# fboehm/DBSLMM

Hardware: AMD Instinct MI355X
Metric: SNPs solved/sec (whole node) + max-|Δβ| vs CPU ref, 1M SNP × 10k indiv (higher is better)
Workload: dtype f64

## Files before the change

dbslmm_amd/_lib.py:

```python
from __future__ import annotations

import ctypes as C
import os

HERE = os.path.dirname(os.path.abspath(__file__))
LIB_PATH = os.path.join(HERE, "libdbslmm_hip.so")

EXPORTS = (
    "dbslmm_abi_version", "dbslmm_ctx_create", "dbslmm_ctx_destroy", "dbslmm_last_error",
    "dbslmm_est", "dbslmm_plan_create", "dbslmm_plan_run", "dbslmm_plan_sync",
    "dbslmm_plan_download", "dbslmm_plan_set_sigma", "dbslmm_plan_destroy", "dbslmm_plan_run_multi",
    "dbslmm_plan_enable_timing", "dbslmm_plan_kernel_ms", "dbslmm_plan_workload",
    "dbslmm_bed_maf", "dbslmm_read_snp_std", "dbslmm_valid_blocks", "dbslmm_plan_variance",
    "dbslmm_ctx_create_multi", "dbslmm_ctx_num_devices", "dbslmm_plan_shard_info",
    "dbslmm_ctx_cache_bed", "dbslmm_ctx_cache_bed_fd", "dbslmm_plan_block_matrix",
    "dbslmm_shard_plan", "dbslmm_plan_create_units", "dbslmm_shard_plan_problem",
    "dbslmm_plan_block_iters", "dbslmm_bed_row_stats", "dbslmm_out_ranges", "dbslmm_plan_score",
    "dbslmm_ld_r2", "dbslmm_clump", "dbslmm_ld_scores", "dbslmm_ldsc_fit",
)

ABI_VERSION = 21
K_UNPACK, K_GRAM, K_CHOL_LARGE, K_CHOL_SMALL, K_CHOL_TILED, K_TRSV, K_PCG, K_PCG_BLOCK = 0, 1, 2, 3, 4, 5, 6, 7
KERNEL_NAMES = ("dbslmm_unpack_stats", "dbslmm_gram", "dbslmm_chol_large", "dbslmm_chol_small",
                "dbslmm_tchol", "dbslmm_trsv", "dbslmm_pcg", "dbslmm_pcg_block")
WORKLOAD_LEN = 22
BLOCK_OK, BLOCK_EMPTY, BLOCK_NOT_PD, BLOCK_MONOMORPHIC, BLOCK_NOT_CONVERGED = 0, 1, 2, 3, 4
SOLVER_AUTO, SOLVER_FACTOR, SOLVER_PCG = 0, 1, 2
SCORE_COUNTS, SCORE_STD = 0, 1


class Options(C.Structure):
    _fields_ = [
        ("tiled_min", C.c_int32), ("gram_big_min", C.c_int32), ("gram_huge_min", C.c_int32),
        ("h2f_mode", C.c_int32), ("cheb_tol", C.c_double), ("lead_min", C.c_int32),
        ("large_cheb", C.c_int32), ("cheb_fused", C.c_int32), ("debug_delay_us", C.c_int32),
        ("debug_stop", C.c_int32), ("sub_split", C.c_int32), ("sub_grid_lead", C.c_int32),
        ("sub_grid_rest", C.c_int32), ("shard_copies", C.c_int32), ("h2f_iter", C.c_int32),
        ("solver", C.c_int32), ("pcg_tol", C.c_double), ("pcg_maxit", C.c_int32),
        ("pcg_whole", C.c_int32), ("stream_out", C.c_int32), ("pcg_block_wgs", C.c_int32),
    ]


class Problem(C.Structure):
    _fields_ = [
        ("bed", C.c_void_p), ("bed_len", C.c_int64), ("n_ref", C.c_int32), ("n_obs", C.c_int32),
        ("sigma_s", C.c_double), ("tau", C.c_double), ("num_block", C.c_int32),
        ("s_ptr", C.c_void_p), ("s_pos", C.c_void_p), ("z_s", C.c_void_p),
        ("l_ptr", C.c_void_p), ("l_pos", C.c_void_p), ("z_l", C.c_void_p),
        ("opts", C.POINTER(Options)),
    ]


class TestPanel(C.Structure):
    _fields_ = [
# ... 94 lines not shown
```

dbslmm_amd/csrc/kernels.hip:

```cpp
#include <hip/hip_runtime.h>
#include <stdint.h>

#include "dims.hpp"

namespace {

typedef int v4i __attribute__((ext_vector_type(4)));
typedef int v16i __attribute__((ext_vector_type(16)));

constexpr int kWave = 64;
constexpr int kLdsStride = 33;

__device__ __forceinline__ void wave_sync() {
    __builtin_amdgcn_fence(__ATOMIC_RELEASE, "wavefront");
    __builtin_amdgcn_wave_barrier();
    __builtin_amdgcn_fence(__ATOMIC_ACQUIRE, "wavefront");
}

__device__ __forceinline__ int wave_sum_i32(int v) {
#pragma unroll
    for (int o = 32; o > 0; o >>= 1) v += __shfl_xor(v, o, kWave);
    return v;
}

// ... 523 lines not shown
                double v = scale * (c * rsd[row0 + li] * rj);
                if (li == lj) v += 1.0 - tau;
                for (int cp = copy_lo(m, tmin, tcopy); cp < copy_hi(m, tmin, tcopy, ncopy); ++cp)
                    M[moff + cp * cstride + static_cast<int64_t>(li) * ld + lj] = v;
            }
        }
    }
}

namespace gram {
constexpr int kHK = 256;
constexpr int kHLdsBytes = 4 * 2 * kHT * (kHK / 4);
static_assert(kKpadAlign == kHK, "kpad: a multiple of the stage");
}

template <int NOP, bool kFull>
__device__ __forceinline__ void gram_huge_dma_loop(const uint8_t* __restrict__ img, int64_t kw,
                                                   const int32_t* __restrict__ slot_pos, int32_t zrow,
                                                   const int64_t (&rbase)[2], const int (&svl)[2], int nst,
                                                   int8_t* lds, int wave, int lane, int wr, int wc,
                                                   uint32_t act, v16f (&acc)[2][4]) {
    typedef __attribute__((address_space(1))) const void* gptr_g;
    typedef __attribute__((address_space(3))) void* lptr_g;
    constexpr int kRowB = 64;
    constexpr int kOpB = gram::kHT * kRowB;
    constexpr int kSlotB = 2 * kOpB;
    const int dr = lane >> 2, dp = lane & 3;
    const uint32_t* gsrc[NOP][2];
#pragma unroll
    for (int op = 0; op < NOP; ++op)
#pragma unroll
        for (int h = 0; h < 2; ++h) {
            const int r = 32 * wave + 16 * h + dr;
            const int q = dp ^ ((r >> 2) & 3);
            const int32_t pos = slot_pos[rbase[op] + min(r, svl[op] - 1)];
            gsrc[op][h] = reinterpret_cast<const uint32_t*>(img) + static_cast<int64_t>(pos < 0 ? zrow : pos) * kw + 4 * q;
        }
    auto issue = [&](int st) {
        int8_t* slot = lds + (st & 3) * kSlotB;
#pragma unroll
        for (int op = 0; op < NOP; ++op)
#pragma unroll
            for (int h = 0; h < 2; ++h)
                __builtin_amdgcn_global_load_lds((gptr_g)(gsrc[op][h] + 16 * st),
                                                 (lptr_g)(slot + op * kOpB + (32 * wave + 16 * h) * kRowB), 16, 0, 0);
    };
    const uint32_t k44 = raw_k44();
    const int rsub = lane & 31, hh = lane >> 5;
    auto roff = [&](int r, int j) { return r * kRowB + 16 * ((2 * j + hh) ^ ((r >> 2) & 3)); };
    auto compute = [&](int st) {
        const int8_t* A = lds + (st & 3) * kSlotB;
        const int8_t* B = NOP == 1 ? A : A + kOpB;
        v4i ar[2][2], br[2][4];
        auto read = [&](int j) {
#pragma unroll
            for (int i = 0; i < 2; ++i) ar[j][i] = *reinterpret_cast<const v4i*>(A + roff(64 * wr + 32 * i + rsub, j));
#pragma unroll
            for (int jj = 0; jj < 4; ++jj) br[j][jj] = *reinterpret_cast<const v4i*>(B + roff(128 * wc + 32 * jj + rsub, j));
        };
        v4i av[2], bv[4];
        auto expand = [&](int j, int e) {
#pragma unroll
            for (int i = 0; i < 2; ++i)
                av[i] = fp4_chunk_raw(static_cast<uint32_t>(ar[j][i][2 * e]), static_cast<uint32_t>(ar[j][i][2 * e + 1]), k44);
#pragma unroll
            for (int jj = 0; jj < 4; ++jj)
                bv[jj] = fp4_chunk_raw(static_cast<uint32_t>(br[j][jj][2 * e]), static_cast<uint32_t>(br[j][jj][2 * e + 1]), k44);
        };
        auto mult = [&]() {
#pragma unroll
            for (int i = 0; i < 2; ++i)
#pragma unroll
                for (int jj = 0; jj < 4; ++jj)
                    if (kFull || (act & (1u << (4 * i + jj)))) acc[i][jj] = mfma_fp4_raw(av[i], bv[jj], acc[i][jj]);
        };
        read(0);
        __builtin_amdgcn_sched_barrier(0);
        expand(0, 0);
        __builtin_amdgcn_sched_barrier(0);
        read(1);
        __builtin_amdgcn_sched_barrier(0);
        mult();
        expand(0, 1);
        mult();
        __builtin_amdgcn_sched_barrier(0);
        expand(1, 0);
        mult();
        expand(1, 1);
        mult();
    };
    auto wait_stage = [&](int ahead) {
        if (ahead >= 2) {
            if constexpr (NOP == 2) asm volatile("s_waitcnt vmcnt(8)" ::: "memory");
            else asm volatile("s_waitcnt vmcnt(4)" ::: "memory");
        } else if (ahead == 1) {
            if constexpr (NOP == 2) asm volatile("s_waitcnt vmcnt(4)" ::: "memory");
            else asm volatile("s_waitcnt vmcnt(2)" ::: "memory");
        } else {
            asm volatile("s_waitcnt vmcnt(0)" ::: "memory");
        }
    };
    for (int st = 0; st < min(3, nst); ++st) issue(st);
    for (int st = 0; st < nst; ++st) {
        wait_stage(min(2, nst - 1 - st));
        __builtin_amdgcn_s_barrier();
        if (st + 3 < nst) issue(st + 3);
        compute(st);
        asm volatile("s_waitcnt lgkmcnt(0)" ::: "memory");
    }
    asm volatile("s_waitcnt vmcnt(0)" ::: "memory");
    __builtin_amdgcn_s_barrier();
}

#define GRAM_HUGE_PARAMS                                                                            \
    const uint8_t* __restrict__ img, int64_t kpad, const int32_t* __restrict__ slot_pos,           \
    int32_t zrow,                                                                                  \
    const GramTile* __restrict__ tiles, int32_t n_tiles,                                           \
    const int32_t* __restrict__ blk_row0, const int32_t* __restrict__ blk_m,                       \
    const int32_t* __restrict__ blk_ld, const int64_t* __restrict__ blk_matoff,                    \
    const int32_t* __restrict__ block_flags,                                                       \
    const double* __restrict__ S, const double* __restrict__ mu, const double* __restrict__ rsd,   \
    double n_ref_d, double pad_k, double tau, double* __restrict__ M,                              \
    int32_t ncopy, int64_t cstride, int32_t tmin, int32_t tcopy, uint16_t* __restrict__ G16,          \
    const int64_t* __restrict__ g16off, const int32_t* __restrict__ g16ld
#define GRAM_HUGE_ARGS img, kpad, slot_pos, zrow, tiles, n_tiles, blk_row0, blk_m, blk_ld, blk_matoff, block_flags, S, \
    mu, rsd, n_ref_d, pad_k, tau, M, ncopy, cstride, tmin, tcopy, G16, g16off, g16ld
__device__ __forceinline__ void gram_huge_body(GRAM_HUGE_PARAMS) {
    using namespace gram;
    extern __shared__ __attribute__((aligned(16))) int8_t hlds[];
    if (static_cast<int>(blockIdx.x) >= n_tiles) return;
    const GramTile tile = tiles[blockIdx.x];
    const int b = tile.block;
    if (b < 0) return;
    const int tid = threadIdx.x, lane = tid & 63, wave = __builtin_amdgcn_readfirstlane(tid >> 6);
    const int row0 = blk_row0[b], m = blk_m[b], ld = blk_ld[b];
    const int64_t moff = blk_matoff[b];
    const bool diag = tile.ti == tile.tj;
    if (block_flags[b] & 1) {
        for (int q = wave; q < 64; q += 8) {
            const int si = q >> 3, sj = q & 7;
            if (diag && sj > si) continue;
            const int r0 = kHT * tile.ti + 32 * si, c0 = kHT * tile.tj + 32 * sj;
            if (r0 >= m || c0 >= m) continue;
            gram_tile32(img, kpad, slot_pos, zrow, row0, m, ld, moff, true, r0, c0, lane, S, mu, rsd, n_ref_d, pad_k,
                        tau, M, ncopy, cstride, tmin, tcopy, nullptr, 0, 0);
        }
        return;
    }
    const int rv = min(kHT, m - kHT * tile.ti), cv = min(kHT, m - kHT * tile.tj);
    const int64_t kw = kpad / 16;
    auto piece_act = [&](int pr, int pc) {
        uint32_t a = 0;
#pragma unroll
        for (int i = 0; i < 2; ++i)
#pragma unroll
            for (int j = 0; j < 4; ++j) {
                const int ri = 64 * pr + 32 * i, cj = 128 * pc + 32 * j;
                if (ri < rv && cj < cv && !(diag && cj >= ri + 32)) a |= 1u << (4 * i + j);
            }
        return a;
    };
    int cnt[8];
#pragma unroll
    for (int q = 0; q < 8; ++q) cnt[q] = __builtin_popcount(piece_act(q >> 1, q & 1));
    const int rank_want = wave < 4 ? wave : 11 - wave;
// ... 3 lines not shown
        int rk = 0;
#pragma unroll
        for (int u = 0; u < 8; ++u) rk += (cnt[u] > cnt[q] || (cnt[u] == cnt[q] && u < q)) ? 1 : 0;
        if (rk == rank_want) pc_sel = q;
    }
    pc_sel = __builtin_amdgcn_readfirstlane(pc_sel);
    const int wr = pc_sel >> 1, wc = pc_sel & 1;
    uint32_t act = piece_act(wr, wc);
    act = __builtin_amdgcn_readfirstlane(act);
    const bool idle = act == 0;
    v16f acc[2][4];
#pragma unroll
    for (int i = 0; i < 2; ++i)
#pragma unroll
        for (int j = 0; j < 4; ++j) acc[i][j] = v16f{0.0f};
    {
        const int nst = static_cast<int>(kpad / kHK);
        const int64_t rbase[2] = {row0 + kHT * tile.ti, row0 + kHT * tile.tj};
        const int svl[2] = {rv, cv};
        if (diag) {
            if (act == 0xFFu) gram_huge_dma_loop<1, true>(img, kw, slot_pos, zrow, rbase, svl, nst, hlds, wave, lane, wr, wc, act, acc);
            else gram_huge_dma_loop<1, false>(img, kw, slot_pos, zrow, rbase, svl, nst, hlds, wave, lane, wr, wc, act, acc);
        } else {
            if (act == 0xFFu) gram_huge_dma_loop<2, true>(img, kw, slot_pos, zrow, rbase, svl, nst, hlds, wave, lane, wr, wc, act, acc);
            else gram_huge_dma_loop<2, false>(img, kw, slot_pos, zrow, rbase, svl, nst, hlds, wave, lane, wr, wc, act, acc);
        }
    }
    double* eRow = reinterpret_cast<double*>(hlds);
    double* eCol = eRow + 2 * kHT;
    {
        const int sop = tid >> 8, k = tid & 255, idx = kHT * (sop ? tile.tj : tile.ti) + k;
        double* e = sop ? eCol : eRow;
        e[k] = idx < m ? S[row0 + idx] : 0.0;
        e[kHT + k] = idx < m ? rsd[row0 + idx] : 0.0;
    }
    __syncthreads();
    if (idle) return;
    int cj[4];
#pragma unroll
    for (int sj = 0; sj < 4; ++sj) cj[sj] = gram_col(eCol[128 * wc + 32 * sj + (lane & 31)]);
    if (G16) {
        const int64_t go = g16off[b], gl = g16ld[b];
#pragma unroll
        for (int si = 0; si < 2; ++si)
#pragma unroll
            for (int r = 0; r < 16; ++r) {
                const int rl = 64 * wr + 32 * si + (r & 3) + 8 * (r >> 2) + 4 * (lane >> 5);
                const int li = kHT * tile.ti + rl;
                if (li >= m) continue;
                const int ri = gram_row(eRow[rl], kpad);
#pragma unroll
                for (int sj = 0; sj < 4; ++sj) {
                    const int lj = kHT * tile.tj + 128 * wc + 32 * sj + (lane & 31);
                    if (!(act & (1u << (4 * si + sj))) || lj >= m) continue;
                    G16[go + li * gl + lj] = static_cast<uint16_t>(gram_exact(acc[si][sj][r], ri, cj[sj]));
                }
            }
        return;
    }
    const double scale = tau / n_ref_d, rn = 1.0 / n_ref_d;
    double Sj[4], rj[4];
#pragma unroll
    for (int sj = 0; sj < 4; ++sj) {
        const int cl = 128 * wc + 32 * sj + (lane & 31);
        Sj[sj] = eCol[cl];
        rj[sj] = eCol[kHT + cl];
    }
#pragma unroll
    for (int si = 0; si < 2; ++si) {
#pragma unroll
        for (int r = 0; r < 16; ++r) {
            const int rl = 64 * wr + 32 * si + (r & 3) + 8 * (r >> 2) + 4 * (lane >> 5);
            const int li = kHT * tile.ti + rl;
            if (li >= m) continue;
            const double Si = eRow[rl], ri = eRow[kHT + rl];
#pragma unroll
            for (int sj = 0; sj < 4; ++sj) {
                const int lj = kHT * tile.tj + 128 * wc + 32 * sj + (lane & 31);
                if (!(act & (1u << (4 * si + sj))) || lj >= m) continue;
                const double c = centre(static_cast<double>(gram_exact(acc[si][sj][r], gram_row(Si, kpad), cj[sj])),
                                        Si * Sj[sj], rn);
                double v = scale * (c * ri * rj[sj]);
                if (li == lj) v += 1.0 - tau;
                for (int cp = copy_lo(m, tmin, tcopy); cp < copy_hi(m, tmin, tcopy, ncopy); ++cp)
                    M[moff + cp * cstride + static_cast<int64_t>(li) * ld + lj] = v;
            }
        }
    }
}

extern "C" __global__ __launch_bounds__(512) void dbslmm_gram_huge(GRAM_HUGE_PARAMS) {
    gram_huge_body(GRAM_HUGE_ARGS);
}

extern "C" __global__ __launch_bounds__(256) void dbslmm_valid_partial(
    const uint8_t* __restrict__ img, int32_t n_ref, int64_t pitch,
    const int64_t* __restrict__ ptr, const int32_t* __restrict__ pos,
    const double* __restrict__ z1, const double* __restrict__ mu, const double* __restrict__ rsd,
    double* __restrict__ partial, int32_t n_chunks, int32_t num_block) {
    __shared__ double red[256 / kWave];
    const int64_t w = static_cast<int64_t>(blockIdx.x) * blockDim.x + threadIdx.x;
    const int64_t n_words = (n_ref + 15) / 16;
// ... 65 lines not shown
```

dbslmm_amd/csrc/plan.hip:

```cpp
#include <hip/hip_runtime.h>
#include <unistd.h>

#include <algorithm>
#include <atomic>
#include <cmath>
#include <cstdio>
#include <cstdlib>
#include <cstring>
#include <initializer_list>
#include <numeric>
#include <string>
#include <memory>
#include <mutex>
#include <thread>
#include <type_traits>
#include <unordered_map>
#include <vector>

#include "../../include/dbslmm_hip.h"
#include "dev_bufs.hpp"
#include "ldsc_fit.hpp"
#include "out_ranges.hpp"
#include "plan_layout.hpp"
#include "host_copy.hpp"
// ... 83 lines not shown
            hipSetDevice(device) == hipSuccess &&
            hipDeviceGetStreamPriorityRange(&prio_lo, &prio_hi) == hipSuccess &&
            hipStreamCreateWithPriority(&c->stream2, hipStreamNonBlocking, prio_hi) == hipSuccess &&
            hipStreamCreateWithPriority(&c->stream3, hipStreamNonBlocking, prio_hi) == hipSuccess &&
            hipStreamCreateWithFlags(&c->stream4, hipStreamNonBlocking) == hipSuccess &&
            hipStreamCreateWithFlags(&c->stream5, hipStreamNonBlocking) == hipSuccess &&
            hipEventCreateWithFlags(&c->fork, hipEventDisableTiming) == hipSuccess &&
            hipEventCreateWithFlags(&c->fork2, hipEventDisableTiming) == hipSuccess &&
            hipEventCreateWithFlags(&c->join4, hipEventDisableTiming) == hipSuccess &&
            hipEventCreateWithFlags(&c->join, hipEventDisableTiming) == hipSuccess &&
            hipEventCreateWithFlags(&c->join3, hipEventDisableTiming) == hipSuccess &&
            set_lds(reinterpret_cast<const void*>(dbslmm_chol_large), kCholLargeLds) &&
            set_lds(reinterpret_cast<const void*>(dbslmm_chol_cheb), kCholChebLds) &&
            set_lds(reinterpret_cast<const void*>(dbslmm_gram_big), gram::kLdsBytes) &&
            set_lds(reinterpret_cast<const void*>(dbslmm_l2_tiles), gram::kLdsBytes) &&
            set_lds(reinterpret_cast<const void*>(dbslmm_gram_huge), gram::kHLdsBytes) &&
            set_lds(reinterpret_cast<const void*>(dbslmm_pcg_block), pcg::block_lds_bytes(pcg::kMaxNC)) &&
            set_lds(reinterpret_cast<const void*>(dbslmm_tchol_region), kRegionLds) &&
            set_lds(reinterpret_cast<const void*>(dbslmm_tchol_panel), kTiledLds) &&
            set_lds(reinterpret_cast<const void*>(dbslmm_tchol_trailing3k16), kTrail3Lds) &&
            set_trsv_lds<1>() && set_trsv_lds<2>();
        DevBufs B(device);
        double* d_warm = nullptr;
        if (c->setup_ok && B.alloc(&d_warm, 1) == hipSuccess) {
            hipLaunchKernelGGL(dbslmm_set_scalar, dim3(1), dim3(1), 0, c->stream2, d_warm, 0.0);
            c->setup_ok = hipStreamSynchronize(c->stream2) == hipSuccess;
        }
    });
    *out = c;
    return DBSLMM_OK;
}
// ... 118 lines not shown

static int record_instants(dbslmm_ctx* ctx, hipEvent_t* ev, std::initializer_list<Ev> ks, hipStream_t st) {
    if (!ev) return DBSLMM_OK;
    for (Ev k : ks) HIP_TRY(ctx, hipEventRecord(ev[k], st));
    return DBSLMM_OK;
}

struct GramOut {
    int32_t ncopy, tmin_copy, tcopy;
    uint16_t* g16;
    const int64_t* off16;
    const int32_t* ld16;
};
enum GramKernel { kGramI8, kGramBig, kGramHuge };
static hipError_t launch_gram(const dbslmm_plan* p, hipStream_t st, GramKernel which, const GramTile* tiles,
                              int32_t nt, const GramOut& o) {
    if (nt <= 0) return hipSuccess;
    struct Shape {
        decltype(&dbslmm_gram_i8) kernel;
        int tiles_per_wg, threads;
        size_t lds;
    };
    static const Shape shapes[] = {{dbslmm_gram_i8, 4, 256, 0},
                                   {dbslmm_gram_big, 1, 256, gram::kLdsBytes},
                                   {dbslmm_gram_huge, 1, 512, gram::kHLdsBytes}};
    const Shape& k = shapes[which];
    hipLaunchKernelGGL(k.kernel, dim3((nt + k.tiles_per_wg - 1) / k.tiles_per_wg), dim3(k.threads), k.lds, st,
                       p->d_img, p->kpad, p->d_slot_pos, p->img.n_rows, tiles, nt, p->d_row0, p->d_m, p->d_ld,
                       p->d_matoff, p->d_flags, p->d_S, p->d_mu, p->d_rsd, static_cast<double>(p->n_ref),
                       static_cast<double>(p->kpad - p->n_ref), p->tau, p->d_M, o.ncopy, p->M_elems, o.tmin_copy,
                       o.tcopy, o.g16, o.off16, o.ld16);
    return hipGetLastError();
}

static void close_run(dbslmm_plan* p, const LastRun& r) { p->last = r; }

#include "route_factor.hip"
#include "route_pcg.hip"

static int run_impl(dbslmm_plan* p, const double* sigmas, int n) {
// ... 86 lines not shown
    static_cast<PlanLayout::Kept&>(*p) = std::move(L.keep);
    p->ctx = ctx;
    p->bufs.device = ctx->device;
    p->n_ref = pr->n_ref;
    p->n_obs = pr->n_obs;
    p->num_block = pr->num_block;
    p->sigma_s = pr->sigma_s;
    p->tau = pr->tau;
    p->bed_len = pr->bed_len;
    p->pcg.g16 = 4 * static_cast<int64_t>(pr->n_ref) <= 65535;
    PlanOptions& o = p->opt;
    o.solver = op.solver;
    o.pcg_fused = op.pcg_whole >= 0;
    o.stream_out = op.stream_out >= 0;
    o.pcg_block_wgs = op.pcg_block_wgs;
    if (op.pcg_tol > 0.0) o.pcg_tol = std::max(1e-15, op.pcg_tol);
    if (op.pcg_maxit > 0) o.pcg_maxit = op.pcg_maxit;
    o.h2f_mode = op.h2f_mode;
    o.cheb_fused = op.cheb_fused == 1;
    o.h2f_cg = op.h2f_iter != 1;
    o.debug_delay_us = op.debug_delay_us;
    o.debug_stop = op.debug_stop;
    if (op.cheb_tol > 0.0) o.cheb_tol = std::max(1e-16, op.cheb_tol);

    hipError_t e = hipSetDevice(ctx->device);
    auto fail = [&](const char* what) {
        ctx->err = std::string(what) + ": " + hipGetErrorString(e);
        dbslmm_plan_destroy(p);
        return DBSLMM_E_HIP;
    };
// ... 22 lines not shown
    up("upload trsv lists", &p->fac.d_tri_f, L.tri_f);
    up("upload trsv lists", &p->fac.d_tri_b, L.tri_b);
    up("upload trsv lists", &p->fac.d_foff, L.foff);
    up("upload trsv lists", &p->fac.d_tb, p->h_tb);
    if (!L.tcheb_list.empty()) up("upload trsv lists", &p->fac.d_tcheb_blocks, L.tcheb_list);
    if (what) return fail(what);
    if ((e = p->bufs.zeroed(&p->fac.d_tflags, p->n_tflags + 3, ctx->stream)) != hipSuccess ||
        (e = p->bufs.zeroed(&p->fac.d_tepi, p->n_tflags, ctx->stream)) != hipSuccess)
        return fail("hipMalloc trsv flags");
    if ((e = p->bufs.alloc(&p->d_S, p->n_slots)) != hipSuccess || (e = p->bufs.alloc(&p->d_mu, p->n_slots)) != hipSuccess ||
        (e = p->bufs.alloc(&p->d_rsd, p->n_slots)) != hipSuccess)
        return fail("hipMalloc stats");
    const size_t nbk = std::max<int32_t>(1, std::max(p->n_nonempty, p->num_block));
    p->nbk = static_cast<int64_t>(nbk);
    if ((e = p->bufs.zeroed(&p->d_flags, nbk, ctx->stream)) != hipSuccess) return fail("hipMalloc flags");
    if ((e = hipStreamSynchronize(ctx->stream)) != hipSuccess) return fail("plan set-up");
    *out = p;
    return DBSLMM_OK;
}

int dbslmm_plan_set_sigma(dbslmm_plan* p, double sigma_s) {
    if (!p) return DBSLMM_E_ARG;
    ARG_CHECK(p->ctx, sigma_s > 0.0 && std::isfinite(sigma_s), "sigma_s must be > 0");
    p->sigma_s = sigma_s;
    if (p->mp)
        for (auto& sh : p->mp->shards) sh.plan->sigma_s = sigma_s;
    return DBSLMM_OK;
}

int dbslmm_plan_enable_timing(dbslmm_plan* p, int enable) {
// ... 214 lines not shown
```

dbslmm_amd/csrc/plan_layout.hpp:

```cpp
#pragma once
#include <stdint.h>

#include <algorithm>
#include <cmath>
#include <numeric>
#include <string>
#include <vector>

#include "../../include/dbslmm_hip.h"
#include "dims.hpp"
#include "out_ranges.hpp"

constexpr int kTiledMinDefault = 384;
constexpr int kTiledMinSmall = 256;
constexpr int kGramBigMinDefault = 96;
constexpr int kGramHugeMinDefault = 384;
constexpr int kTChebMaxM = 4096;
constexpr int kLeadMinDefault = 1536;
constexpr int kXcd = 8;
constexpr int kSuper = 2;
constexpr int kWideSuper = 4;
constexpr int kWideMin = 4096;
constexpr int kTiledMaxM = 255 * 128;
constexpr int kGramSq = 4;
// ... 211 lines not shown
        }
    }
    if (G > 0) sync(kTlWait, 2 * G - 1, 0);
}

inline int build_plan_layout(const dbslmm_problem& pr, const dbslmm_options& op, int n_cu, PlanLayout& out,
                             std::string& err) {
    if (!(op.tiled_min >= 0 && op.gram_big_min >= 0 && op.gram_huge_min >= 0 &&
          (op.h2f_mode == 0 || op.h2f_mode == 1) && op.cheb_tol >= 0.0 &&
          (op.large_cheb == 0 || op.large_cheb == -1) && (op.cheb_fused == 0 || op.cheb_fused == 1) &&
          op.debug_delay_us >= -100000 && op.debug_delay_us <= 100000 &&
          (op.debug_stop == 0 || op.debug_stop == 1) && op.sub_split >= -1 && op.sub_split <= 2 &&
          op.sub_grid_lead >= 0 && op.sub_grid_rest >= 0 && op.shard_copies >= 0 &&
          op.shard_copies <= 64 && op.h2f_iter >= 0 && op.h2f_iter <= 2 && op.solver >= 0 &&
          op.solver <= 2 && op.pcg_tol >= 0.0 && op.pcg_maxit >= 0 && op.stream_out >= -1 &&
          op.stream_out <= 1 && op.pcg_block_wgs >= 0)) {
        err = "bad dbslmm_options";
        return DBSLMM_E_ARG;
    }
    out = PlanLayout{};
    PlanLayout::Kept& k = out.keep;
    const bool has_l = pr.l_ptr != nullptr;
    const int64_t n_snp_bed = (pr.bed_len - 3) / bed_row_bytes(pr.n_ref);
    k.n_s = pr.s_ptr[pr.num_block];
    k.n_l = has_l ? pr.l_ptr[pr.num_block] : 0;
    k.kpad = round_up(pr.n_ref, gram::kKpadAlign);

    std::vector<int32_t>&slot_pos = out.slot_pos, &slot_block = out.slot_block, &slot_out = k.h_slot_out;
    std::vector<int32_t>&row0 = k.h_row0, &mv = k.h_m, &msv = k.h_ms, &ldv = k.h_ld, &blk_id = k.h_blk_id;
    std::vector<double>& z = out.z;
    std::vector<int64_t>& matoff = k.h_matoff;
// ... 265 lines not shown
```

dbslmm_amd/csrc/plan_state.hpp:

```cpp
#pragma once

namespace {
enum Ev {
    kEvStart,
    kEvStatsEnd,
    kEvGramEnd,
    kEvLargeEnd,
    kEvSmallBegin,
    kEvSmallEnd,
    kEvTiledBegin,
    kEvEnd,
    kEvTiledEnd,
    kEvLeadGramBegin,
    kEvLeadGramEnd,
    kEvRestEnd,
    kEvCount,
    kEvPcgBlockBegin = kEvLargeEnd,
    kEvPcgBlockEnd = kEvSmallBegin,
};
static_assert(sizeof(v4i) == kRowEntryBytes, "one row-table entry");
struct PanelImage {
    std::shared_ptr<uint8_t> mem;
    int64_t pitch = 0;
    int32_t n_rows = 0, n_ref = 0;
// ... 30 lines not shown
    int device_index = 0;
    int copy = -1;
    std::vector<int32_t> blocks;
    std::vector<int64_t> s_idx, l_idx;
    std::vector<int> run_copies;
    std::vector<double> dl_s, dl_l;
    std::vector<int32_t> dl_st;
};
struct dbslmm_mplan {
    std::vector<DeviceShard> shards;
    int32_t n_copies = 1;
    bool partial = false;
    std::vector<int32_t> unit_device;
};

struct PlanOptions {
    int32_t solver = 0;
    double pcg_tol = 1e-12;
    int32_t pcg_maxit = 1000;
    bool pcg_fused = true;
    int32_t pcg_block_wgs = 0;
    bool stream_out = true;
    int32_t h2f_mode = 0;
    double cheb_tol = 1e-9;
    bool cheb_fused = false;
    bool h2f_cg = false;
    int32_t debug_delay_us = 0;
    int32_t debug_stop = 0;
};

struct LastRun {
    bool ran = false;
    bool stopped = false;
    double sigma_run = 0.0;
    int32_t var_copy = 0;
    int32_t score_copies = 0;
// ... 107 lines not shown
    PlanOptions opt;
    LastRun last;
    int64_t n_runs = 0;
    bool force_factor = false;
    DevBufs bufs;
    PanelImage img;
    const uint8_t* d_img = nullptr;
    int32_t *d_slot_pos = nullptr, *d_slot_block = nullptr, *d_slot_out = nullptr;
    double *d_z = nullptr, *d_S = nullptr, *d_mu = nullptr, *d_rsd = nullptr, *d_y = nullptr;
    int32_t *d_flags = nullptr, *d_status = nullptr, *d_order = nullptr, *d_blk_id = nullptr;
    int32_t *d_row0 = nullptr, *d_m = nullptr, *d_ms = nullptr, *d_ld = nullptr;
    int64_t* d_matoff = nullptr;
    GramTile* d_tiles = nullptr;
    GramTile* d_btiles = nullptr;
    GramTile* d_htiles = nullptr;
    double* d_M = nullptr;
    double *d_beta_s = nullptr, *d_beta_l = nullptr;
    double* d_dshift = nullptr;
    int32_t n_copies = 0;
    int32_t m_copies = 0;
    int64_t nbk = 1;
    PinnedBuf pin;
    EventList dl_ev;
    PcgState pcg;
    StreamOut so;
    FactorState fac;
    Timing tm;
};

struct CopyView {
// ... 68 lines not shown
```

dbslmm_amd/csrc/route_factor.hip:

```cpp

struct TSeq {
    hipStream_t chain, bulk;
    EventList* tev;
};
static TSeq seq_main(dbslmm_plan* p) { return TSeq{p->ctx->stream2, p->ctx->stream3, &p->fac.tev}; }
static TSeq seq_rest(dbslmm_plan* p) { return TSeq{p->ctx->stream4, p->ctx->stream5, &p->fac.tev_rest}; }

static void debug_spin(const dbslmm_plan* p, hipStream_t st, int side) {
    const int32_t d = p->opt.debug_delay_us;
    if (d == 0 || (d > 0) != (side > 0)) return;
    const int64_t ticks = 100 * static_cast<int64_t>(d > 0 ? d : -d);
    hipLaunchKernelGGL(dbslmm_debug_spin, dim3(1), dim3(64), 0, st, ticks);
}

static int enqueue_tiled(dbslmm_plan* p, double isn, const std::vector<TLaunch>& tl, const int32_t* d_tlist,
                         int copy, const TSeq& sq) {
    dbslmm_ctx* ctx = p->ctx;
    const CopyView v = copy_view(p, copy);
    const chol::TiledArgs ta{v.M, p->d_row0, p->d_m, p->d_ms, p->d_ld, p->d_matoff, p->d_blk_id, p->d_z,
                             p->d_slot_out, p->d_rsd, v.dshift, isn, v.y, v.beta_s, v.beta_l, v.status,
                             p->n_nonempty, p->M_elems, p->n_slots, p->n_s, p->n_l, p->nbk};
    int nev = 0;
    for (const TLaunch& L : tl)
        if (L.kind == kTlRecord) nev = std::max(nev, L.step + 1);
// ... 452 lines not shown
            hipLaunchKernelGGL(dbslmm_set_scalar, dim3(1), dim3(1), 0, s, p->d_dshift + c, dshift);
        }
        if (cheb) {
            const int rc = cheb_prepare(p, cp, s);
            if (rc != DBSLMM_OK) return rc;
        }
    }
    const GramOut go{n, tmin_copy, tcopy, nullptr, nullptr, nullptr};
    HIP_TRY(ctx, launch_gram(p, s, kGramHuge, p->d_htiles, p->n_htiles_lead, go));
    if (ev) HIP_TRY(ctx, hipEventRecord(ev[kEvLeadGramEnd], s));
    if (lead) {
        HIP_TRY(ctx, hipEventRecord(ctx->fork, s));
        debug_spin(p, s, 1);
    }
    if (ev) HIP_TRY(ctx, hipEventRecord(ev[kEvStatsEnd], s));
    HIP_TRY(ctx, launch_gram(p, s, kGramHuge, p->d_htiles + p->n_htiles_lead, p->n_htiles_tiled - p->n_htiles_lead, go));
    const bool early = p->early_fork && p->n_nonempty > 0;
    if (early) {
        HIP_TRY(ctx, hipEventRecord(ctx->fork2, s));
        HIP_TRY(ctx, hipStreamWaitEvent(lead ? ctx->stream4 : ctx->stream2, ctx->fork2, 0));
    }
    HIP_TRY(ctx, launch_gram(p, s, kGramI8, p->d_tiles, p->n_tiles, go));
    HIP_TRY(ctx, launch_gram(p, s, kGramHuge, p->d_htiles + p->n_htiles_tiled, p->n_htiles - p->n_htiles_tiled, go));
    HIP_TRY(ctx, launch_gram(p, s, kGramBig, p->d_btiles, p->n_btiles, go));
    if (ev) HIP_TRY(ctx, hipEventRecord(ev[kEvGramEnd], s));
    if (p->opt.debug_stop == 1) {
        if (const int rc = record_instants(ctx, ev, kEvAfterGram, s)) return rc;
        LastRun r = p->last;
        r.ran = true;
        r.stopped = true;
        r.pcg_ran = false;
        r.pcg_pending_var = false;
        close_run(p, r);
        return DBSLMM_OK;
    }
    if (p->n_nonempty > 0) {
        if (!early) {
            HIP_TRY(ctx, hipEventRecord(ctx->fork2, s));
// ... 140 lines not shown
```

include/dbslmm_hip.h:

```cpp
#ifndef DBSLMM_HIP_H_
#define DBSLMM_HIP_H_

#include <stdint.h>

#ifdef __cplusplus
extern "C" {
#endif

#define DBSLMM_ABI_VERSION 21

enum {
    DBSLMM_OK = 0,
    DBSLMM_E_ARG = -1,
    DBSLMM_E_HIP = -2,
    DBSLMM_E_STATE = -3
};

enum {
    DBSLMM_BLOCK_OK = 0,
    DBSLMM_BLOCK_EMPTY = 1,
    DBSLMM_BLOCK_NOT_PD = 2,
    DBSLMM_BLOCK_MONOMORPHIC = 3,
    DBSLMM_BLOCK_NOT_CONVERGED = 4
};
// ... 11 lines not shown
    int32_t large_cheb;
    int32_t cheb_fused;
    int32_t debug_delay_us;
    int32_t debug_stop;
    int32_t sub_split;
    int32_t sub_grid_lead;
    int32_t sub_grid_rest;
    int32_t shard_copies;
    int32_t h2f_iter;
    int32_t solver;
    double pcg_tol;
    int32_t pcg_maxit;
    int32_t pcg_whole;
    int32_t stream_out;
    int32_t pcg_block_wgs;
} dbslmm_options;

typedef struct dbslmm_problem {
    const uint8_t* bed;
    int64_t bed_len;
    int32_t n_ref;
    int32_t n_obs;
    double sigma_s;
    double tau;
    int32_t num_block;
    const int64_t* s_ptr;
    const int32_t* s_pos;
    const double* z_s;
    const int64_t* l_ptr;
    const int32_t* l_pos;
// ... 126 lines not shown
```

Baseline: 160.8 million.

## Make huge Gram kernel persistent with per-XCD tile queues and cross-tile DMA prefetch

Converts the huge Gram tile kernel from one workgroup per tile into a persistent kernel, with the grid capped at the CU count or a new gram_huge_wgs option. Workgroups pull tiles from per-XCD atomic ticket counters and prefetch the next tile's first DMA stages into LDS while the current tile's epilogue runs. It also skips padded K sub-steps in the final stage. The aim is to hide launch, tail and pipeline-fill costs, in exchange for atomic counters, a self-reset protocol and more complex synchronisation that risks races.

```diff
diff --git a/dbslmm_amd/_lib.py b/dbslmm_amd/_lib.py
--- a/dbslmm_amd/_lib.py
+++ b/dbslmm_amd/_lib.py
@@ -19,7 +19,7 @@
     "dbslmm_ld_r2", "dbslmm_clump", "dbslmm_ld_scores", "dbslmm_ldsc_fit",
 )
 
-ABI_VERSION = 21
+ABI_VERSION = 22
 K_UNPACK, K_GRAM, K_CHOL_LARGE, K_CHOL_SMALL, K_CHOL_TILED, K_TRSV, K_PCG, K_PCG_BLOCK = 0, 1, 2, 3, 4, 5, 6, 7
 KERNEL_NAMES = ("dbslmm_unpack_stats", "dbslmm_gram", "dbslmm_chol_large", "dbslmm_chol_small",
                 "dbslmm_tchol", "dbslmm_trsv", "dbslmm_pcg", "dbslmm_pcg_block")
@@ -38,6 +38,7 @@
         ("sub_grid_rest", C.c_int32), ("shard_copies", C.c_int32), ("h2f_iter", C.c_int32),
         ("solver", C.c_int32), ("pcg_tol", C.c_double), ("pcg_maxit", C.c_int32),
         ("pcg_whole", C.c_int32), ("stream_out", C.c_int32), ("pcg_block_wgs", C.c_int32),
+        ("gram_huge_wgs", C.c_int32),
     ]
 
 
diff --git a/dbslmm_amd/csrc/kernels.hip b/dbslmm_amd/csrc/kernels.hip
--- a/dbslmm_amd/csrc/kernels.hip
+++ b/dbslmm_amd/csrc/kernels.hip
@@ -561,41 +561,58 @@
 static_assert(kKpadAlign == kHK, "kpad: a multiple of the stage");
 }
 
+namespace gram {
+constexpr int kHRowB = 64;
+constexpr int kHOpB = kHT * kHRowB;
+constexpr int kHSlotB = 2 * kHOpB;
+constexpr int kHLdsAll = kHLdsBytes + 16;
+}
+
+__device__ __forceinline__ void huge_slot_rows(const int32_t* __restrict__ slot_pos, const int64_t (&rbase)[2],
+                                               const int (&svl)[2], int wave, int lane, int32_t (&pos)[4]) {
+#pragma unroll
+    for (int op = 0; op < 2; ++op)
+#pragma unroll
+        for (int h = 0; h < 2; ++h)
+            pos[2 * op + h] = slot_pos[rbase[op] + min(32 * wave + 16 * h + (lane >> 2), svl[op] - 1)];
+}
+__device__ __forceinline__ void huge_dma_src(const uint8_t* __restrict__ img, int64_t kw, int32_t zrow,
+                                             const int32_t (&pos)[4], int wave, int lane,
+                                             const uint32_t* (&gsrc)[2][2]) {
+#pragma unroll
+    for (int op = 0; op < 2; ++op)
+#pragma unroll
+        for (int h = 0; h < 2; ++h) {
+            const int r = 32 * wave + 16 * h + (lane >> 2);
+            const int q = (lane & 3) ^ ((r >> 2) & 3);
+            const int32_t ps = pos[2 * op + h];
+            gsrc[op][h] = reinterpret_cast<const uint32_t*>(img) + static_cast<int64_t>(ps < 0 ? zrow : ps) * kw + 4 * q;
+        }
+}
+template <int NOP>
+__device__ __forceinline__ void huge_dma_issue(const uint32_t* (&gsrc)[2][2], int st, int8_t* lds, int wave) {
+    typedef __attribute__((address_space(1))) const void* gptr_g;
+    typedef __attribute__((address_space(3))) void* lptr_g;
+    int8_t* slot = lds + (st & 3) * gram::kHSlotB;
+#pragma unroll
+    for (int op = 0; op < NOP; ++op)
+#pragma unroll
+        for (int h = 0; h < 2; ++h)
+            __builtin_amdgcn_global_load_lds((gptr_g)(gsrc[op][h] + 16 * st),
+                                             (lptr_g)(slot + op * gram::kHOpB + (32 * wave + 16 * h) * gram::kHRowB), 16, 0, 0);
+}
+
 template <int NOP, bool kFull>
-__device__ __forceinline__ void gram_huge_dma_loop(const uint8_t* __restrict__ img, int64_t kw,
-                                                   const int32_t* __restrict__ slot_pos, int32_t zrow,
-                                                   const int64_t (&rbase)[2], const int (&svl)[2], int nst,
+__device__ __forceinline__ void gram_huge_dma_loop(const uint32_t* (&gsrc)[2][2], bool pre, int nst, int nk,
                                                    int8_t* lds, int wave, int lane, int wr, int wc,
                                                    uint32_t act, v16f (&acc)[2][4]) {
-    typedef __attribute__((address_space(1))) const void* gptr_g;
-    typedef __attribute__((address_space(3))) void* lptr_g;
-    constexpr int kRowB = 64;
-    constexpr int kOpB = gram::kHT * kRowB;
-    constexpr int kSlotB = 2 * kOpB;
-    const int dr = lane >> 2, dp = lane & 3;
-    const uint32_t* gsrc[NOP][2];
-#pragma unroll
-    for (int op = 0; op < NOP; ++op)
-#pragma unroll
-        for (int h = 0; h < 2; ++h) {
-            const int r = 32 * wave + 16 * h + dr;
-            const int q = dp ^ ((r >> 2) & 3);
-            const int32_t pos = slot_pos[rbase[op] + min(r, svl[op] - 1)];
-            gsrc[op][h] = reinterpret_cast<const uint32_t*>(img) + static_cast<int64_t>(pos < 0 ? zrow : pos) * kw + 4 * q;
-        }
-    auto issue = [&](int st) {
-        int8_t* slot = lds + (st & 3) * kSlotB;
-#pragma unroll
-        for (int op = 0; op < NOP; ++op)
-#pragma unroll
-            for (int h = 0; h < 2; ++h)
-                __builtin_amdgcn_global_load_lds((gptr_g)(gsrc[op][h] + 16 * st),
-                                                 (lptr_g)(slot + op * kOpB + (32 * wave + 16 * h) * kRowB), 16, 0, 0);
-    };
+    constexpr int kRowB = gram::kHRowB, kOpB = gram::kHOpB, kSlotB = gram::kHSlotB;
+    auto issue = [&](int st) { huge_dma_issue<NOP>(gsrc, st, lds, wave); };
     const uint32_t k44 = raw_k44();
     const int rsub = lane & 31, hh = lane >> 5;
     auto roff = [&](int r, int j) { return r * kRowB + 16 * ((2 * j + hh) ^ ((r >> 2) & 3)); };
-    auto compute = [&](int st) {
+    auto compute = [&](int st, auto last_tag) {
+        constexpr bool kLast = decltype(last_tag)::value;
         const int8_t* A = lds + (st & 3) * kSlotB;
         const int8_t* B = NOP == 1 ? A : A + kOpB;
         v4i ar[2][2], br[2][4];
@@ -625,16 +642,22 @@
         __builtin_amdgcn_sched_barrier(0);
         expand(0, 0);
         __builtin_amdgcn_sched_barrier(0);
-        read(1);
+        if (!kLast || nk > 2) read(1);
         __builtin_amdgcn_sched_barrier(0);
         mult();
-        expand(0, 1);
-        mult();
+        if (!kLast || nk > 1) {
+            expand(0, 1);
+            mult();
+        }
         __builtin_amdgcn_sched_barrier(0);
-        expand(1, 0);
-        mult();
-        expand(1, 1);
-        mult();
+        if (!kLast || nk > 2) {
+            expand(1, 0);
+            mult();
+        }
+        if (!kLast || nk > 3) {
+            expand(1, 1);
+            mult();
+        }
     };
     auto wait_stage = [&](int ahead) {
         if (ahead >= 2) {
@@ -647,14 +670,19 @@
             asm volatile("s_waitcnt vmcnt(0)" ::: "memory");
         }
     };
-    for (int st = 0; st < min(3, nst); ++st) issue(st);
-    for (int st = 0; st < nst; ++st) {
-        wait_stage(min(2, nst - 1 - st));
+    if (!pre)
+        for (int st = 0; st < min(3, nst); ++st) issue(st);
+    for (int st = 0; st < nst - 1; ++st) {
+        wait_stage(pre && st == 0 ? 0 : min(2, nst - 1 - st));
         __builtin_amdgcn_s_barrier();
         if (st + 3 < nst) issue(st + 3);
-        compute(st);
+        compute(st, std::false_type{});
         asm volatile("s_waitcnt lgkmcnt(0)" ::: "memory");
     }
+    wait_stage(0);
+    __builtin_amdgcn_s_barrier();
+    compute(nst - 1, std::true_type{});
+    asm volatile("s_waitcnt lgkmcnt(0)" ::: "memory");
     asm volatile("s_waitcnt vmcnt(0)" ::: "memory");
     __builtin_amdgcn_s_barrier();
 }
@@ -669,21 +697,82 @@
     const double* __restrict__ S, const double* __restrict__ mu, const double* __restrict__ rsd,   \
     double n_ref_d, double pad_k, double tau, double* __restrict__ M,                              \
     int32_t ncopy, int64_t cstride, int32_t tmin, int32_t tcopy, uint16_t* __restrict__ G16,          \
-    const int64_t* __restrict__ g16off, const int32_t* __restrict__ g16ld
+    const int64_t* __restrict__ g16off, const int32_t* __restrict__ g16ld, int32_t* __restrict__ ctr
 #define GRAM_HUGE_ARGS img, kpad, slot_pos, zrow, tiles, n_tiles, blk_row0, blk_m, blk_ld, blk_matoff, block_flags, S, \
-    mu, rsd, n_ref_d, pad_k, tau, M, ncopy, cstride, tmin, tcopy, G16, g16off, g16ld
+    mu, rsd, n_ref_d, pad_k, tau, M, ncopy, cstride, tmin, tcopy, G16, g16off, g16ld, ctr
+
+struct HugeTile {
+    int b, ti, tj, row0, m, miss;
+};
+template <typename T>
+__device__ __forceinline__ T huge_uniform(const T* p) {
+    return *(const __attribute__((address_space(4))) T*)p;
+}
+
 __device__ __forceinline__ void gram_huge_body(GRAM_HUGE_PARAMS) {
     using namespace gram;
     extern __shared__ __attribute__((aligned(16))) int8_t hlds[];
-    if (static_cast<int>(blockIdx.x) >= n_tiles) return;
-    const GramTile tile = tiles[blockIdx.x];
-    const int b = tile.block;
-    if (b < 0) return;
-    const int tid = threadIdx.x, lane = tid & 63, wave = __builtin_amdgcn_readfirstlane(tid >> 6);
-    const int row0 = blk_row0[b], m = blk_m[b], ld = blk_ld[b];
-    const int64_t moff = blk_matoff[b];
+    auto tkw = [&](int i) -> int& {
+        int off = kHLdsBytes + 4 * i;
+        asm volatile("" : "+s"(off));
+        return *reinterpret_cast<int*>(hlds + off);
+    };
+    const int tid0 = threadIdx.x, wave = __builtin_amdgcn_readfirstlane(tid0 >> 6);
+    const int64_t kw = kpad / 16;
+    const int nst = static_cast<int>(kpad / kHK);
+    const int rem = kHK - static_cast<int>(pad_k);
+    const int nk = rem > 0 ? 1 + (rem > 32) + (rem > 128) + (rem > 160) : 4;
+    const int64_t kmul = kpad - 64 * (4 - nk);
+    const int grid = static_cast<int>(gridDim.x), wg = static_cast<int>(blockIdx.x);
+    const int qstep = min(grid, kXcd);
+    for (int qu = wg % qstep; qu < kXcd; qu += qstep) {
+    auto fetch = [&](int ticket) {
+        HugeTile t{-1, 0, 0, 0, 0, 0};
+        const int e = __builtin_amdgcn_readfirstlane(ticket) * kXcd + qu;
+        if (e < n_tiles) {
+            const v4i rec = huge_uniform(reinterpret_cast<const v4i*>(tiles + e));
+            const GramTile g{rec[0], rec[1], rec[2], rec[3]};
+            if (g.block >= 0) t = HugeTile{g.block, g.ti, g.tj, huge_uniform(blk_row0 + g.block), huge_uniform(blk_m + g.block),
+                                               huge_uniform(block_flags + g.block) & 1};
+            else t = HugeTile{0, 0, 0, 0, 0, 2};
+        }
+        return t;
+    };
+    auto slot_rows = [&](const HugeTile& t, int lane, int32_t (&pos)[4]) {
+        const int64_t rbase[2] = {t.row0 + kHT * t.ti, t.row0 + kHT * t.tj};
+        const int svl[2] = {min(kHT, t.m - kHT * t.ti), min(kHT, t.m - kHT * t.tj)};
+        huge_slot_rows(slot_pos, rbase, svl, wave, lane, pos);
+    };
+    __syncthreads();
+    if (tid0 == 0)
+        for (int i = 0; i < 3; ++i) tkw(i == 2 ? 1 : 2 + i) = atomicAdd(&ctr[qu], 1);
+    __syncthreads();
+    HugeTile cur = fetch(tkw(2)), nxt = fetch(tkw(3));
+    const uint32_t* gsrc[2][2] = {{nullptr, nullptr}, {nullptr, nullptr}};
+    int32_t posn[4] = {0, 0, 0, 0};
+    {
+        int tidp = tid0;
+        asm volatile("" : "+v"(tidp));
+        if (cur.b >= 0 && !cur.miss) {
+            int32_t pos[4];
+            slot_rows(cur, tidp & 63, pos);
+            huge_dma_src(img, kw, zrow, pos, wave, tidp & 63, gsrc);
+        }
+        if (nxt.b >= 0 && !nxt.miss) slot_rows(nxt, tidp & 63, posn);
+    }
+#pragma unroll
+    for (int i = 0; i < 4; ++i) asm volatile("" : "+v"(posn[i]));
+    bool pre = false;
+    for (int t = 0; cur.b >= 0; ++t) {
+    int tid = tid0;
+    asm volatile("" : "+v"(tid));
+    const int lane = tid & 63;
+    const int b = cur.b, row0 = cur.row0, m = cur.m;
+    const GramTile tile{b, cur.ti, cur.tj, 0};
     const bool diag = tile.ti == tile.tj;
-    if (block_flags[b] & 1) {
+    if (cur.miss == 1) {
+        const int ld = blk_ld[b];
+        const int64_t moff = blk_matoff[b];
         for (int q = wave; q < 64; q += 8) {
             const int si = q >> 3, sj = q & 7;
             if (diag && sj > si) continue;
@@ -692,10 +781,9 @@
             gram_tile32(img, kpad, slot_pos, zrow, row0, m, ld, moff, true, r0, c0, lane, S, mu, rsd, n_ref_d, pad_k,
                         tau, M, ncopy, cstride, tmin, tcopy, nullptr, 0, 0);
         }
-        return;
-    }
+    }
+    if (cur.miss) __syncthreads();
     const int rv = min(kHT, m - kHT * tile.ti), cv = min(kHT, m - kHT * tile.tj);
-    const int64_t kw = kpad / 16;
     auto piece_act = [&](int pr, int pc) {
         uint32_t a = 0;
 #pragma unroll
@@ -729,55 +817,77 @@
     for (int i = 0; i < 2; ++i)
 #pragma unroll
         for (int j = 0; j < 4; ++j) acc[i][j] = v16f{0.0f};
-    {
-        const int nst = static_cast<int>(kpad / kHK);
-        const int64_t rbase[2] = {row0 + kHT * tile.ti, row0 + kHT * tile.tj};
-        const int svl[2] = {rv, cv};
+    if (!cur.miss) {
         if (diag) {
-            if (act == 0xFFu) gram_huge_dma_loop<1, true>(img, kw, slot_pos, zrow, rbase, svl, nst, hlds, wave, lane, wr, wc, act, acc);
-            else gram_huge_dma_loop<1, false>(img, kw, slot_pos, zrow, rbase, svl, nst, hlds, wave, lane, wr, wc, act, acc);
+            if (act == 0xFFu) gram_huge_dma_loop<1, true>(gsrc, pre, nst, nk, hlds, wave, lane, wr, wc, act, acc);
+            else gram_huge_dma_loop<1, false>(gsrc, pre, nst, nk, hlds, wave, lane, wr, wc, act, acc);
         } else {
-            if (act == 0xFFu) gram_huge_dma_loop<2, true>(img, kw, slot_pos, zrow, rbase, svl, nst, hlds, wave, lane, wr, wc, act, acc);
-            else gram_huge_dma_loop<2, false>(img, kw, slot_pos, zrow, rbase, svl, nst, hlds, wave, lane, wr, wc, act, acc);
-        }
-    }
-    double* eRow = reinterpret_cast<double*>(hlds);
+            if (act == 0xFFu) gram_huge_dma_loop<2, true>(gsrc, pre, nst, nk, hlds, wave, lane, wr, wc, act, acc);
+            else gram_huge_dma_loop<2, false>(gsrc, pre, nst, nk, hlds, wave, lane, wr, wc, act, acc);
+        }
+    }
+    int tidh = tid0;
+    asm volatile("" : "+v"(tidh));
+    const int laneh = tidh & 63;
+    double eS = 0.0, eR = 0.0;
+    if (!cur.miss) {
+        const int sop = tidh >> 8, k = tidh & 255, idx = kHT * (sop ? tile.tj : tile.ti) + k;
+        eS = idx < m ? S[row0 + idx] : 0.0;
+        eR = idx < m ? rsd[row0 + idx] : 0.0;
+    }
+    pre = nxt.b >= 0 && !nxt.miss;
+    if (pre) {
+        huge_dma_src(img, kw, zrow, posn, wave, laneh, gsrc);
+        if (nxt.ti == nxt.tj)
+            for (int st = 0; st < min(3, nst); ++st) huge_dma_issue<1>(gsrc, st, hlds, wave);
+        else
+            for (int st = 0; st < min(3, nst); ++st) huge_dma_issue<2>(gsrc, st, hlds, wave);
+    }
+    const HugeTile nn = fetch(tkw((t + 1) & 1));
+    if (nn.b >= 0 && !nn.miss) slot_rows(nn, laneh, posn);
+    int tk3 = 0;
+    if (tidh == 0) tk3 = atomicAdd(&ctr[qu], 1);
+    double* eRow = reinterpret_cast<double*>(hlds + 3 * kHSlotB);
     double* eCol = eRow + 2 * kHT;
-    {
-        const int sop = tid >> 8, k = tid & 255, idx = kHT * (sop ? tile.tj : tile.ti) + k;
-        double* e = sop ? eCol : eRow;
-        e[k] = idx < m ? S[row0 + idx] : 0.0;
-        e[kHT + k] = idx < m ? rsd[row0 + idx] : 0.0;
-    }
-    __syncthreads();
-    if (idle) return;
+    if (!cur.miss) {
+        double* e = (tidh >> 8) ? eCol : eRow;
+        e[tidh & 255] = eS;
+        e[kHT + (tidh & 255)] = eR;
+        asm volatile("s_waitcnt lgkmcnt(0)" ::: "memory");
+        __builtin_amdgcn_s_barrier();
+        asm volatile("" ::: "memory");
+    }
+    if (!cur.miss && !idle) {
     int cj[4];
 #pragma unroll
-    for (int sj = 0; sj < 4; ++sj) cj[sj] = gram_col(eCol[128 * wc + 32 * sj + (lane & 31)]);
+    for (int sj = 0; sj < 4; ++sj) cj[sj] = gram_col(eCol[128 * wc + 32 * sj + (laneh & 31)]);
     if (G16) {
-        const int64_t go = g16off[b], gl = g16ld[b];
+        const int64_t go = huge_uniform(g16off + b), gl = huge_uniform(g16ld + b);
 #pragma unroll
         for (int si = 0; si < 2; ++si)
 #pragma unroll
             for (int r = 0; r < 16; ++r) {
-                const int rl = 64 * wr + 32 * si + (r & 3) + 8 * (r >> 2) + 4 * (lane >> 5);
+                const int rl = 64 * wr + 32 * si + (r & 3) + 8 * (r >> 2) + 4 * (laneh >> 5);
                 const int li = kHT * tile.ti + rl;
                 if (li >= m) continue;
-                const int ri = gram_row(eRow[rl], kpad);
+                const int ri = gram_row(eRow[rl], kmul);
 #pragma unroll
                 for (int sj = 0; sj < 4; ++sj) {
-                    const int lj = kHT * tile.tj + 128 * wc + 32 * sj + (lane & 31);
+                    const int lj = kHT * tile.tj + 128 * wc + 32 * sj + (laneh & 31);
                     if (!(act & (1u << (4 * si + sj))) || lj >= m) continue;
                     G16[go + li * gl + lj] = static_cast<uint16_t>(gram_exact(acc[si][sj][r], ri, cj[sj]));
                 }
             }
-        return;
-    }
-    const double scale = tau / n_ref_d, rn = 1.0 / n_ref_d;
+    } else {
+    const int ld = huge_uniform(blk_ld + b);
+    const int64_t moff = huge_uniform(blk_matoff + b);
+    double nrd = n_ref_d;
+    asm volatile("" : "+s"(nrd));
+    const double scale = tau / nrd, rn = 1.0 / nrd;
     double Sj[4], rj[4];
 #pragma unroll
     for (int sj = 0; sj < 4; ++sj) {
-        const int cl = 128 * wc + 32 * sj + (lane & 31);
+        const int cl = 128 * wc + 32 * sj + (laneh & 31);
         Sj[sj] = eCol[cl];
         rj[sj] = eCol[kHT + cl];
     }
@@ -785,15 +895,15 @@
     for (int si = 0; si < 2; ++si) {
 #pragma unroll
         for (int r = 0; r < 16; ++r) {
-            const int rl = 64 * wr + 32 * si + (r & 3) + 8 * (r >> 2) + 4 * (lane >> 5);
+            const int rl = 64 * wr + 32 * si + (r & 3) + 8 * (r >> 2) + 4 * (laneh >> 5);
             const int li = kHT * tile.ti + rl;
             if (li >= m) continue;
             const double Si = eRow[rl], ri = eRow[kHT + rl];
 #pragma unroll
             for (int sj = 0; sj < 4; ++sj) {
-                const int lj = kHT * tile.tj + 128 * wc + 32 * sj + (lane & 31);
+                const int lj = kHT * tile.tj + 128 * wc + 32 * sj + (laneh & 31);
                 if (!(act & (1u << (4 * si + sj))) || lj >= m) continue;
-                const double c = centre(static_cast<double>(gram_exact(acc[si][sj][r], gram_row(Si, kpad), cj[sj])),
+                const double c = centre(static_cast<double>(gram_exact(acc[si][sj][r], gram_row(Si, kmul), cj[sj])),
                                         Si * Sj[sj], rn);
                 double v = scale * (c * ri * rj[sj]);
                 if (li == lj) v += 1.0 - tau;
@@ -801,6 +911,22 @@
                     M[moff + cp * cstride + static_cast<int64_t>(li) * ld + lj] = v;
             }
         }
+    }
+    }
+    }
+    asm volatile("s_waitcnt vmcnt(0)" ::: "memory");
+#pragma unroll
+    for (int i = 0; i < 4; ++i) asm volatile("" : "+v"(posn[i]));
+    if (tidh == 0) tkw(t & 1) = tk3;
+    asm volatile("s_waitcnt lgkmcnt(0)" ::: "memory");
+    cur = nxt;
+    nxt = nn;
+    }
+    }
+    if (tid0 == 0) {
+        __threadfence();
+        if (atomicAdd(&ctr[kXcd], 1) == grid - 1)
+            for (int i = 0; i <= kXcd; ++i) atomicExch(&ctr[i], 0);
     }
 }
 
diff --git a/dbslmm_amd/csrc/plan.hip b/dbslmm_amd/csrc/plan.hip
--- a/dbslmm_amd/csrc/plan.hip
+++ b/dbslmm_amd/csrc/plan.hip
@@ -121,7 +121,7 @@
             set_lds(reinterpret_cast<const void*>(dbslmm_chol_cheb), kCholChebLds) &&
             set_lds(reinterpret_cast<const void*>(dbslmm_gram_big), gram::kLdsBytes) &&
             set_lds(reinterpret_cast<const void*>(dbslmm_l2_tiles), gram::kLdsBytes) &&
-            set_lds(reinterpret_cast<const void*>(dbslmm_gram_huge), gram::kHLdsBytes) &&
+            set_lds(reinterpret_cast<const void*>(dbslmm_gram_huge), gram::kHLdsAll) &&
             set_lds(reinterpret_cast<const void*>(dbslmm_pcg_block), pcg::block_lds_bytes(pcg::kMaxNC)) &&
             set_lds(reinterpret_cast<const void*>(dbslmm_tchol_region), kRegionLds) &&
             set_lds(reinterpret_cast<const void*>(dbslmm_tchol_panel), kTiledLds) &&
@@ -270,16 +270,24 @@
 };
 enum GramKernel { kGramI8, kGramBig, kGramHuge };
 static hipError_t launch_gram(const dbslmm_plan* p, hipStream_t st, GramKernel which, const GramTile* tiles,
-                              int32_t nt, const GramOut& o) {
+                              int32_t nt, const GramOut& o, int cset = 0) {
     if (nt <= 0) return hipSuccess;
+    if (which == kGramHuge) {
+        int grid = std::min(p->ctx->n_cu, nt);
+        if (p->opt.gram_huge_wgs > 0) grid = std::min(grid, p->opt.gram_huge_wgs);
+        hipLaunchKernelGGL(dbslmm_gram_huge, dim3(grid), dim3(512), gram::kHLdsAll, st, p->d_img, p->kpad,
+                           p->d_slot_pos, p->img.n_rows, tiles, nt, p->d_row0, p->d_m, p->d_ld, p->d_matoff, p->d_flags,
+                           p->d_S, p->d_mu, p->d_rsd, static_cast<double>(p->n_ref),
+                           static_cast<double>(p->kpad - p->n_ref), p->tau, p->d_M, o.ncopy, p->M_elems, o.tmin_copy,
+                           o.tcopy, o.g16, o.off16, o.ld16, p->d_gram_ctr + cset * kGramCtrStride);
+        return hipGetLastError();
+    }
     struct Shape {
         decltype(&dbslmm_gram_i8) kernel;
         int tiles_per_wg, threads;
         size_t lds;
     };
-    static const Shape shapes[] = {{dbslmm_gram_i8, 4, 256, 0},
-                                   {dbslmm_gram_big, 1, 256, gram::kLdsBytes},
-                                   {dbslmm_gram_huge, 1, 512, gram::kHLdsBytes}};
+    static const Shape shapes[] = {{dbslmm_gram_i8, 4, 256, 0}, {dbslmm_gram_big, 1, 256, gram::kLdsBytes}};
     const Shape& k = shapes[which];
     hipLaunchKernelGGL(k.kernel, dim3((nt + k.tiles_per_wg - 1) / k.tiles_per_wg), dim3(k.threads), k.lds, st,
                        p->d_img, p->kpad, p->d_slot_pos, p->img.n_rows, tiles, nt, p->d_row0, p->d_m, p->d_ld,
@@ -396,6 +404,7 @@
     o.pcg_fused = op.pcg_whole >= 0;
     o.stream_out = op.stream_out >= 0;
     o.pcg_block_wgs = op.pcg_block_wgs;
+    o.gram_huge_wgs = op.gram_huge_wgs;
     if (op.pcg_tol > 0.0) o.pcg_tol = std::max(1e-15, op.pcg_tol);
     if (op.pcg_maxit > 0) o.pcg_maxit = op.pcg_maxit;
     o.h2f_mode = op.h2f_mode;
@@ -448,6 +457,8 @@
     const size_t nbk = std::max<int32_t>(1, std::max(p->n_nonempty, p->num_block));
     p->nbk = static_cast<int64_t>(nbk);
     if ((e = p->bufs.zeroed(&p->d_flags, nbk, ctx->stream)) != hipSuccess) return fail("hipMalloc flags");
+    if ((e = p->bufs.zeroed(&p->d_gram_ctr, kGramCtrSets * kGramCtrStride, ctx->stream)) != hipSuccess)
+        return fail("hipMalloc gram counters");
     if ((e = hipStreamSynchronize(ctx->stream)) != hipSuccess) return fail("plan set-up");
     *out = p;
     return DBSLMM_OK;
diff --git a/dbslmm_amd/csrc/plan_layout.hpp b/dbslmm_amd/csrc/plan_layout.hpp
--- a/dbslmm_amd/csrc/plan_layout.hpp
+++ b/dbslmm_amd/csrc/plan_layout.hpp
@@ -249,7 +249,7 @@
           op.sub_grid_lead >= 0 && op.sub_grid_rest >= 0 && op.shard_copies >= 0 &&
           op.shard_copies <= 64 && op.h2f_iter >= 0 && op.h2f_iter <= 2 && op.solver >= 0 &&
           op.solver <= 2 && op.pcg_tol >= 0.0 && op.pcg_maxit >= 0 && op.stream_out >= -1 &&
-          op.stream_out <= 1 && op.pcg_block_wgs >= 0)) {
+          op.stream_out <= 1 && op.pcg_block_wgs >= 0 && op.gram_huge_wgs >= 0)) {
         err = "bad dbslmm_options";
         return DBSLMM_E_ARG;
     }
diff --git a/dbslmm_amd/csrc/plan_state.hpp b/dbslmm_amd/csrc/plan_state.hpp
--- a/dbslmm_amd/csrc/plan_state.hpp
+++ b/dbslmm_amd/csrc/plan_state.hpp
@@ -68,12 +68,16 @@
     std::vector<int32_t> unit_device;
 };
 
+constexpr int kGramCtrSets = 3, kGramCtrStride = 16;
+static_assert(kXcd + 1 <= kGramCtrStride, "a counter set: one word per queue and the leave count");
+
 struct PlanOptions {
     int32_t solver = 0;
     double pcg_tol = 1e-12;
     int32_t pcg_maxit = 1000;
     bool pcg_fused = true;
     int32_t pcg_block_wgs = 0;
+    int32_t gram_huge_wgs = 0;
     bool stream_out = true;
     int32_t h2f_mode = 0;
     double cheb_tol = 1e-9;
@@ -211,6 +215,7 @@
     GramTile* d_tiles = nullptr;
     GramTile* d_btiles = nullptr;
     GramTile* d_htiles = nullptr;
+    int32_t* d_gram_ctr = nullptr;
     double* d_M = nullptr;
     double *d_beta_s = nullptr, *d_beta_l = nullptr;
     double* d_dshift = nullptr;
diff --git a/dbslmm_amd/csrc/route_factor.hip b/dbslmm_amd/csrc/route_factor.hip
--- a/dbslmm_amd/csrc/route_factor.hip
+++ b/dbslmm_amd/csrc/route_factor.hip
@@ -490,14 +490,14 @@
         debug_spin(p, s, 1);
     }
     if (ev) HIP_TRY(ctx, hipEventRecord(ev[kEvStatsEnd], s));
-    HIP_TRY(ctx, launch_gram(p, s, kGramHuge, p->d_htiles + p->n_htiles_lead, p->n_htiles_tiled - p->n_htiles_lead, go));
+    HIP_TRY(ctx, launch_gram(p, s, kGramHuge, p->d_htiles + p->n_htiles_lead, p->n_htiles_tiled - p->n_htiles_lead, go, 1));
     const bool early = p->early_fork && p->n_nonempty > 0;
     if (early) {
         HIP_TRY(ctx, hipEventRecord(ctx->fork2, s));
         HIP_TRY(ctx, hipStreamWaitEvent(lead ? ctx->stream4 : ctx->stream2, ctx->fork2, 0));
     }
     HIP_TRY(ctx, launch_gram(p, s, kGramI8, p->d_tiles, p->n_tiles, go));
-    HIP_TRY(ctx, launch_gram(p, s, kGramHuge, p->d_htiles + p->n_htiles_tiled, p->n_htiles - p->n_htiles_tiled, go));
+    HIP_TRY(ctx, launch_gram(p, s, kGramHuge, p->d_htiles + p->n_htiles_tiled, p->n_htiles - p->n_htiles_tiled, go, 2));
     HIP_TRY(ctx, launch_gram(p, s, kGramBig, p->d_btiles, p->n_btiles, go));
     if (ev) HIP_TRY(ctx, hipEventRecord(ev[kEvGramEnd], s));
     if (p->opt.debug_stop == 1) {
diff --git a/include/dbslmm_hip.h b/include/dbslmm_hip.h
--- a/include/dbslmm_hip.h
+++ b/include/dbslmm_hip.h
@@ -7,7 +7,7 @@
 extern "C" {
 #endif
 
-#define DBSLMM_ABI_VERSION 21
+#define DBSLMM_ABI_VERSION 22
 
 enum {
     DBSLMM_OK = 0,
@@ -49,6 +49,7 @@
     int32_t pcg_whole;
     int32_t stream_out;
     int32_t pcg_block_wgs;
+    int32_t gram_huge_wgs;
 } dbslmm_options;
 
 typedef struct dbslmm_problem {
```

New measurement: 162.8 million (median of 2 runs). About the same (+1.3%).
